# MasterBin-IIAU/UNINEXT

Measured on NVIDIA H100. Metric: msdeformattn_fwd_bwd_gsamples_per_s, higher is better.
Workload: dtype f32

## Files before the change

uninext_b200/csrc/msda_cabi.cu:

```cuda
#include <type_traits>

#include "../../include/msda_b200.h"
#include "msda_det.cuh"
#include "msda_generic.cuh"
#include "msda_host.cuh"
#include "msda_region.cuh"
#include "msda_slab.cuh"
#include "msda_tmem.cuh"
#include "msda_tiled.cuh"

std::atomic<uint64_t> msda_host::g_launches{0};

namespace {

using namespace msda_host;

struct Dims { int N, S, M, D, L, Lq, P; };

int check_dims(const Dims &d) {
    if (d.N <= 0 || d.S <= 0 || d.M <= 0 || d.D <= 0 || d.L <= 0 || d.Lq <= 0 || d.P <= 0) return MSDA_E_BADARG;
    if ((long long)d.S >= (1ll << 30)) return MSDA_E_TOOLARGE;
    if ((long long)d.N * d.Lq * d.M >= (1ll << 40)) return MSDA_E_TOOLARGE;
    return 0;
}

struct Knobs {
    std::atomic<int> v[MSDA_KNOB_COUNT];
    std::atomic<int> epoch{1};
    Knobs() {
        v[MSDA_KNOB_SLAB].store(env_int("MSDA_SLAB", -1));
        v[MSDA_KNOB_BWD_WIN_ROWS].store(env_int("MSDA_BWD_WIN_ROWS", -1));
        v[MSDA_KNOB_BWD_LIST_CAP].store(env_int("MSDA_BWD_LIST_CAP", 48));
        v[MSDA_KNOB_FWD_SLAB_CTAS].store(env_int("MSDA_FWD_SLAB_CTAS", 2));
        v[MSDA_KNOB_F32_VEC8_FWD].store(env_int("MSDA_F32_VEC8_FWD", 0));
        v[MSDA_KNOB_F32_VEC8_BWD].store(env_int("MSDA_F32_VEC8_BWD", 0));
        v[MSDA_KNOB_BF16_FINE_ROWS].store(env_int("MSDA_BF16_FINE_ROWS", 0));
        v[MSDA_KNOB_BF16_PACKED_FWD].store(env_int("MSDA_BF16_PACKED_FWD", 0));
        v[MSDA_KNOB_ZERO_FILL].store(env_int("MSDA_ZERO_FILL", 2));
        v[MSDA_KNOB_REGION_BWD].store(env_int("MSDA_REGION_BWD", -1));
    }
};
Knobs &knobs() { static Knobs k; return k; }
int knob(int i) { return knobs().v[i].load(std::memory_order_relaxed); }

cudaError_t zero_fill(void *p, size_t bytes, cudaStream_t st, bool *pdl = nullptr) {
    if (pdl) *pdl = false;
    const int mode = knob(MSDA_KNOB_ZERO_FILL);
    if (mode <= 0 || bytes < (1u << 16) || !aligned16(p) || (bytes & 15u)) return cudaMemsetAsync(p, 0, bytes, st);
    const unsigned long long n16 = bytes >> 4;
    msda::msda_zero_fill<<<capped_grid((long long)n16, 256, 8), 256, 0, st>>>(static_cast<uint4 *>(p), n16);
    const cudaError_t err = cudaGetLastError();
    if (pdl && mode >= 2 && err == cudaSuccess) {
        cudaStreamCaptureStatus cap = cudaStreamCaptureStatusNone;
        *pdl = cudaStreamIsCapturing(st, &cap) == cudaSuccess && cap == cudaStreamCaptureStatusNone;
    }
    return err;
}

bool fast_ok(int dtype_bytes, int D, int L, int P) {
    if (L > msda::kMaxLevels || L * P > 32) return false;
    if (dtype_bytes == 4) return D == 16 || D == 32 || D == 64;
    if (dtype_bytes == 2) return D == 32 || D == 64;
    return false;
}

bool use_fast(int dtype_bytes, const Dims &d) {
    return fast_ok(dtype_bytes, d.D, d.L, d.P) && (long long)d.N * d.Lq * d.M < (1ll << 31);
}

unsigned num_pairs(const Dims &d) { return (unsigned)((long long)d.N * d.Lq * d.M); }

template <typename T, class F>
cudaError_t route_tiled(const Dims &d, F f) {
    using L16 = std::integral_constant<int, 16>;
    using L32 = std::integral_constant<int, 32>;
    const bool lp16 = d.L * d.P <= 16;
    switch (d.D) {
        case 16:
            if constexpr (sizeof(T) == 4) return lp16 ? f(L16{}, L16{}) : f(L16{}, L32{});
            break;
        case 32: return lp16 ? f(L32{}, L16{}) : f(L32{}, L32{});
        case 64: return lp16 ? f(std::integral_constant<int, 64>{}, L16{}) : f(std::integral_constant<int, 64>{}, L32{});
    }
    return cudaErrorInvalidValue;
}

template <typename K>
int resident_ctas(K kernel) {
    int per_sm = 0;
    if (cudaOccupancyMaxActiveBlocksPerMultiprocessor(&per_sm, kernel, msda::kTiledThreads, 0) != cudaSuccess || per_sm < 1)
        per_sm = 1;
    return per_sm * num_sms();
}

int allow_patches() {
    static const int v = env_flag("MSDA_PATCHES") == 1;
    return v;
}

bool use_tma_staging(const Dims &d) {
    static const bool off = env_flag("MSDA_NO_TMA") == 1;
    return !off && !allow_patches() && ((d.L * d.P) % 4 == 0);
}

bool use_split(unsigned npairs) {
    static const int force = env_flag("MSDA_SPLIT");
    if (force >= 0) return force == 1;
    return npairs <= (unsigned)num_sms() * 56u;
}

constexpr int kFwdMinCtas = 4, kBwdMinCtas = 2;


template <typename T> struct FwdVec { static constexpr int v = 16 / sizeof(T); };
template <typename T> struct BwdVec { static constexpr int v = 4; };

template <typename K, typename... Args>
cudaError_t launch_after_fill(K kern, int grid, size_t smem, cudaStream_t st, bool pdl, Args... args) {
    if (pdl) {
        cudaLaunchConfig_t cfg = {};
        cfg.gridDim = dim3((unsigned)grid);
        cfg.blockDim = dim3(msda::kTiledThreads);
        cfg.dynamicSmemBytes = smem;
        cfg.stream = st;
        cudaLaunchAttribute attr[1];
        attr[0].id = cudaLaunchAttributeProgrammaticStreamSerialization;
        attr[0].val.programmaticStreamSerializationAllowed = 1;
        cfg.attrs = attr;
        cfg.numAttrs = 1;
        const cudaError_t e = cudaLaunchKernelEx(&cfg, kern, args...);
        return e != cudaSuccess ? e : cudaGetLastError();
    }
    kern<<<grid, msda::kTiledThreads, smem, st>>>(args...);
    return cudaGetLastError();
}

template <typename K, typename... Args>
cudaError_t launch_tiled(K kern, PerDevice<int> &slots, unsigned npairs, unsigned iter_pairs, bool pdl, cudaStream_t st,
                         Args... args) {
    const unsigned n = (unsigned)slots.get([&](int) { return resident_ctas(kern); });
    const unsigned tiles_ub = (npairs + iter_pairs - 1) / iter_pairs;
    g_launches.fetch_add(1, std::memory_order_relaxed);
    return launch_after_fill(kern, (int)(tiles_ub < n ? tiles_ub : n), 0, st, pdl, args...);
}

template <typename T, int D, int LP_MAX, int VEC = FwdVec<T>::v>
cudaError_t launch_fwd(const T *value, const int64_t *shapes, const int64_t *lsi, const float *loc, const float *attn,
                       const Dims &d, T *out, cudaStream_t st) {
    using Shape = msda::TiledShape<VEC, D, LP_MAX, false>;
    constexpr bool kCanStage = (LP_MAX <= 16);
    constexpr bool kCanSplit = Shape::kCanSplit;
    constexpr bool kCanPack = sizeof(T) == 2 && VEC == 8;
    const unsigned npairs = num_pairs(d);
    const bool split = kCanSplit && use_split(npairs);
    const bool tma = !split && kCanStage && use_tma_staging(d);
    const bool packed = kCanPack && !split && knob(MSDA_KNOB_BF16_PACKED_FWD) == 1;
    static decltype(&msda::msda_fwd_tiled<T, VEC, D, LP_MAX, kFwdMinCtas, false, false>) const kern[] = {
        msda::msda_fwd_tiled<T, VEC, D, LP_MAX, kFwdMinCtas, false, kCanSplit>,
        msda::msda_fwd_tiled<T, VEC, D, LP_MAX, kFwdMinCtas, kCanStage, false>,
        msda::msda_fwd_tiled<T, VEC, D, LP_MAX, kFwdMinCtas, false, false>,
        msda::msda_fwd_tiled<T, VEC, D, LP_MAX, kFwdMinCtas, kCanStage, false, kCanPack>,
        msda::msda_fwd_tiled<T, VEC, D, LP_MAX, kFwdMinCtas, false, false, kCanPack>};
    static PerDevice<int> slots[5];
    const int k = split ? 0 : (packed ? 3 : 1) + (tma ? 0 : 1);
    return launch_tiled(kern[k], slots[k], npairs, split ? msda::TiledShape<VEC, D, LP_MAX, kCanSplit>::kIterPairs
                                                         : Shape::kIterPairs,
                        false, st, value, shapes, lsi, loc, attn, d.N, d.S, d.M, d.L, d.Lq, d.P, npairs, allow_patches(), out);
}

template <typename T, int D, int LP_MAX, int VEC = BwdVec<T>::v, bool NORED = false>
cudaError_t launch_bwd(const T *grad_out, const T *value, const int64_t *shapes, const int64_t *lsi, const float *loc,
                       const float *attn, const Dims &d, float *gv, float *gl, float *ga, bool pdl, cudaStream_t st) {
    using Shape = msda::TiledShape<VEC, D, LP_MAX, false>;
    constexpr bool kCanStage = (LP_MAX <= 16);
    constexpr bool kCanSplit = Shape::kCanSplit;
    const unsigned npairs = num_pairs(d);
    const bool split = kCanSplit && use_split(npairs);
    const bool tma = !split && kCanStage && use_tma_staging(d);
    static decltype(&msda::msda_bwd_tiled<T, VEC, D, LP_MAX, kBwdMinCtas, false, false, false, NORED>) const kern[] = {
        msda::msda_bwd_tiled<T, VEC, D, LP_MAX, kBwdMinCtas, false, kCanSplit, false, NORED>,
        msda::msda_bwd_tiled<T, VEC, D, LP_MAX, kBwdMinCtas, kCanStage, false, false, NORED>,
        msda::msda_bwd_tiled<T, VEC, D, LP_MAX, kBwdMinCtas, false, false, false, NORED>};
    static PerDevice<int> slots[3];
    const int k = split ? 0 : tma ? 1 : 2;
    return launch_tiled(kern[k], slots[k], npairs, split ? msda::TiledShape<VEC, D, LP_MAX, kCanSplit>::kIterPairs
                                                         : Shape::kIterPairs,
                        pdl, st, grad_out, value, shapes, lsi, loc, attn, d.N, d.S, d.M, d.L, d.Lq, d.P, npairs,
                        allow_patches(), gv, gl, ga, (__nv_bfloat16 *)nullptr, 0);
}


bool use_slab(const Dims &d, const void *value, const void *out) {
    if (d.D != 32 || d.L * d.P > 16 || d.L > msda::kMaxLevels) return false;
    if ((reinterpret_cast<uintptr_t>(value) & 31u) || !aligned16(out)) return false;
    return knob(MSDA_KNOB_SLAB) == 1;
}

template <typename T>
cudaError_t launch_fwd_slab(const T *value, const int64_t *shapes, const int64_t *lsi, const float *loc, const float *attn,
                            const Dims &d, T *out, cudaStream_t st) {
    const int sms = num_sms();
    if (knob(MSDA_KNOB_FWD_SLAB_CTAS) == 1)
        return launch(msda::msda_fwd_slab<T, 16, 1>, sms, msda::kSlabThreads, 0, st, value, shapes, lsi, loc, attn, d.N,
                      d.S, d.M, d.L, d.Lq, d.P, sms, out);
    return launch(msda::msda_fwd_slab<T, 16, 2>, sms * 2, msda::kSlabThreads, 0, st, value, shapes, lsi, loc, attn, d.N,
                  d.S, d.M, d.L, d.Lq, d.P, sms, out);
}

struct Window { int rows, cap; };

template <auto Kernel, class Smem, class Fit>
cudaError_t bwd_window(int cap_max, Smem smem, Fit fit, Window &w) {
    static PerDevice<uint64_t> cache;
    const uint64_t epoch = (uint32_t)knobs().epoch.load(std::memory_order_acquire);
    cudaError_t e = cudaSuccess;
    const uint64_t v = cache.get([&](int dev) -> uint64_t {
        int cap = knob(MSDA_KNOB_BWD_LIST_CAP) & ~1;
        if (cap < 8) cap = 8;
        if (cap > cap_max) cap = cap_max;
        int max_optin = 0;
        cudaDeviceGetAttribute(&max_optin, cudaDevAttrMaxSharedMemoryPerBlockOptin, dev);
        cudaFuncAttributes fa{};
        cudaFuncGetAttributes(&fa, Kernel);
        const long long fixed = (long long)smem(0, cap) + (long long)fa.sharedSizeBytes + 64;
        int rows = fit((int)((max_optin - fixed) / 128));
        if (rows < 0) rows = 0;
        if ((e = opt_in_smem<Kernel>((int)smem(rows, cap))) != cudaSuccess) return 0;
        return epoch << 32 | (uint64_t)rows << 16 | (uint64_t)cap;
    }, [&](uint64_t c) { return c >> 32 == epoch; });
    w = Window{(int)(v >> 16 & 0xffff), (int)(v & 0xffff)};
    return e;
}

template <typename T>
cudaError_t launch_bwd_slab(const T *grad_out, const T *value, const int64_t *shapes, const int64_t *lsi, const float *loc,
                            const float *attn, const Dims &d, float *gv, float *gl, float *ga, cudaStream_t st) {
    constexpr auto kern = msda::msda_bwd_slab<T, 16>;
    const auto smem = [](int rows, int cap) { return msda::bwd_slab_smem_bytes(rows, cap); };
    Window w;
    const cudaError_t e = bwd_window<kern>(1 << 30, smem, [](int rows) {
        const int want = knob(MSDA_KNOB_BWD_WIN_ROWS);
        return want >= 0 && want < rows ? want : rows;
    }, w);
    if (e != cudaSuccess) return e;
    const int sms = num_sms();
    return launch(kern, sms, msda::kSlabThreads, smem(w.rows, w.cap), st, grad_out, value, shapes, lsi, loc, attn, d.N,
                  d.S, d.M, d.L, d.Lq, d.P, sms, w.rows, w.cap, gv, gl, ga);
}

cudaError_t launch_bwd_mixed(const __nv_bfloat16 *go, const __nv_bfloat16 *value, const int64_t *shapes, const int64_t *lsi,
                             const float *loc, const float *attn, const Dims &d, float *scratch, __nv_bfloat16 *gv16,
                             float *gl, float *ga, int fine_min_rows, cudaStream_t st) {
    using T = __nv_bfloat16;
    constexpr int VEC = 4, DD = 32, LP_MAX = 16;
    const unsigned npairs = num_pairs(d);
    static decltype(&msda::msda_bwd_tiled<T, VEC, DD, LP_MAX, kBwdMinCtas, false, false, true>) const kern[] = {
        msda::msda_bwd_tiled<T, VEC, DD, LP_MAX, kBwdMinCtas, true, false, true>,
        msda::msda_bwd_tiled<T, VEC, DD, LP_MAX, kBwdMinCtas, false, false, true>};
    static PerDevice<int> slots[2];
    const int k = use_tma_staging(d) ? 0 : 1;
    return launch_tiled(kern[k], slots[k], npairs, msda::TiledShape<VEC, DD, LP_MAX, false>::kIterPairs, false, st, go,
                        value, shapes, lsi, loc, attn, d.N, d.S, d.M, d.L, d.Lq, d.P, npairs, allow_patches(), scratch,
                        gl, ga, gv16, fine_min_rows);
}

template <typename T>
cudaError_t launch_bwd_tmem(const T *grad_out, const T *value, const int64_t *shapes, const int64_t *lsi, const float *loc,
                            const float *attn, const Dims &d, float *gv, float *gl, float *ga, cudaStream_t st) {
    constexpr auto kern = msda::msda_bwd_tmem<T, 16>;
    const auto smem = [](int rows, int cap) { return msda::bwd_tmem_smem_bytes(cap, rows); };
    Window w;
    const cudaError_t e = bwd_window<kern>(128, smem, [](int rows) { return rows & ~(msda::kTmCons - 1); }, w);
    if (e != cudaSuccess) return e;
    const int sms = num_sms();
    return launch(kern, sms, msda::kTmThreads, smem(w.rows, w.cap), st, grad_out, value, shapes, lsi, loc, attn, d.N, d.S,
                  d.M, d.L, d.Lq, d.P, sms, w.cap, w.rows, gv, gl, ga);
}

bool use_region(const Dims &d) {
    return knob(MSDA_KNOB_REGION_BWD) != 0 && d.D == 32 && d.L * d.P <= 16 && d.L <= msda::kMaxLevels && d.Lq == d.S &&
           !use_split(num_pairs(d));
}

cudaError_t launch_bwd_region(const float *go, const float *value, const int64_t *shapes, const int64_t *lsi,
                              const float *loc, const float *attn, const Dims &d, float *gv, float *gl, float *ga,
                              bool pdl, cudaStream_t st) {
    constexpr auto tap = msda::msda_bwd_region<msda::kRegionEdge, msda::kRegionHalo>;
    constexpr auto gvk = msda::msda_region_grad_value_pass<msda::kRegionEdge, msda::kRegionHalo>;
    constexpr size_t tap_smem = msda::region_tap_smem_bytes(), gv_smem = msda::region_gv_smem_bytes();
    if (const cudaError_t e = opt_in_smem<gvk>((int)gv_smem)) return e;
    const auto resident = [](auto kern, size_t smem) {
        int per_sm = 0;
        if (cudaOccupancyMaxActiveBlocksPerMultiprocessor(&per_sm, kern, msda::kTiledThreads, smem) != cudaSuccess || per_sm < 1)
            per_sm = 1;
        return per_sm * num_sms();
    };
    static PerDevice<int> tap_slots, gv_slots;
    const int tap_grid = tap_slots.get([&](int) { return resident(tap, tap_smem); });
    const int gv_grid = gv_slots.get([&](int) { return resident(gvk, gv_smem); });
    const unsigned npairs = num_pairs(d);
    const int tma = use_tma_staging(d) ? 1 : 0;
    g_launches.fetch_add(2, std::memory_order_relaxed);
    cudaError_t e = launch_after_fill(tap, tap_grid, tap_smem, st, pdl, go, value, shapes, lsi, loc, attn, d.N, d.S, d.M,
                                      d.L, d.Lq, d.P, npairs, tma, gl, ga);
    if (e != cudaSuccess) return e;
    cudaStreamCaptureStatus cap = cudaStreamCaptureStatusNone;
    const bool chain = cudaStreamIsCapturing(st, &cap) == cudaSuccess && cap == cudaStreamCaptureStatusNone;
    return launch_after_fill(gvk, gv_grid, gv_smem, st, chain, go, shapes, lsi, loc, attn, d.N, d.S, d.M, d.L, d.Lq, d.P,
                             npairs, gv);
}

template <typename T>
cudaError_t fwd_fast(const T *value, const int64_t *shapes, const int64_t *lsi, const float *loc, const float *attn,
                     const Dims &d, T *out, cudaStream_t st) {
    if (use_slab(d, value, out)) return launch_fwd_slab<T>(value, shapes, lsi, loc, attn, d, out, st);
    if constexpr (sizeof(T) == 4) {
        if (knob(MSDA_KNOB_F32_VEC8_FWD) == 1 && d.L * d.P <= 16 && (d.D == 32 || d.D == 64) &&
            !(reinterpret_cast<uintptr_t>(value) & 31u))
            return d.D == 32 ? launch_fwd<T, 32, 16, 8>(value, shapes, lsi, loc, attn, d, out, st)
                             : launch_fwd<T, 64, 16, 8>(value, shapes, lsi, loc, attn, d, out, st);
    }
    return route_tiled<T>(d, [&](auto D, auto LP) {
        return launch_fwd<T, decltype(D)::value, decltype(LP)::value>(value, shapes, lsi, loc, attn, d, out, st);
    });
}

template <typename T>
cudaError_t bwd_fast(const T *go, const T *value, const int64_t *shapes, const int64_t *lsi, const float *loc,
                     const float *attn, const Dims &d, float *gv, float *gl, float *ga, bool pdl, cudaStream_t st) {
    const int LP = d.L * d.P;
    if (knob(MSDA_KNOB_SLAB) == 2 && d.D == 32 && LP <= 16 && d.L <= msda::kMaxLevels)
        return launch_bwd_tmem<T>(go, value, shapes, lsi, loc, attn, d, gv, gl, ga, st);
    if (use_slab(d, value, gv)) return launch_bwd_slab<T>(go, value, shapes, lsi, loc, attn, d, gv, gl, ga, st);
    if constexpr (sizeof(T) == 4) {
        if (knob(MSDA_KNOB_F32_VEC8_BWD) == 1 && LP <= 16 && d.D == 32 &&
            !((reinterpret_cast<uintptr_t>(value) | reinterpret_cast<uintptr_t>(go)) & 31u))
            return launch_bwd<T, 32, 16, 8>(go, value, shapes, lsi, loc, attn, d, gv, gl, ga, pdl, st);
        if (use_region(d)) return launch_bwd_region(go, value, shapes, lsi, loc, attn, d, gv, gl, ga, pdl, st);
    }
    return route_tiled<T>(d, [&](auto D, auto LPM) {
        return launch_bwd<T, decltype(D)::value, decltype(LPM)::value>(go, value, shapes, lsi, loc, attn, d, gv, gl, ga,
                                                                       pdl, st);
    });
}

template <typename T, typename TL>
cudaError_t fwd_generic(const T *value, const int64_t *shapes, const int64_t *lsi, const TL *loc, const TL *attn,
                        const Dims &d, T *out, cudaStream_t st) {
    const long long total = (long long)d.N * d.Lq * d.M * d.D;
    return launch(msda::msda_fwd_generic<T, TL>, capped_grid(total, 256, 32), 256, 0, st, value, shapes, lsi, loc, attn,
                  d.S, d.M, d.D, d.L, d.Lq, d.P, total, out);
}

template <typename T, typename TL, typename GA, bool NORED = false>
cudaError_t bwd_generic(const T *go, const T *value, const int64_t *shapes, const int64_t *lsi, const TL *loc,
                        const TL *attn, const Dims &d, GA *gv, TL *gl, TL *ga, cudaStream_t st) {
    const long long npairs = (long long)d.N * d.Lq * d.M;
    int threads = ((d.D + 31) / 32) * 32;
    if (threads > 256) threads = 256;
    return launch(msda::msda_bwd_generic<T, TL, GA, NORED>, capped_grid(npairs, 1, 64), threads, 0, st, go, value, shapes,
                  lsi, loc, attn, d.S, d.M, d.D, d.L, d.Lq, d.P, npairs, gv, gl, ga);
}

cudaError_t round_to_bf16(const float *gv32, uint16_t *gv, size_t nval, cudaStream_t st) {
    return launch(msda::msda_f32_to_bf16, capped_grid((long long)nval, 256, 16), 256, 0, st, gv32,
                  reinterpret_cast<__nv_bfloat16 *>(gv), (long long)nval);
}

template <class A> struct Elem { using type = A; };
template <> struct Elem<uint16_t> { using type = __nv_bfloat16; };

#define MSDA_CHECK_PTRS(ALIGNED, ...)                                    \
    bool ALIGNED = true;                                                 \
    do {                                                                 \
        const void *ptrs_[] = {__VA_ARGS__};                             \
        for (const void *p_ : ptrs_) {                                   \
            if (p_ == nullptr) return MSDA_E_BADARG;                     \
            ALIGNED = ALIGNED && aligned16(p_);                          \
        }                                                                \
    } while (0)

template <class A, class TL>
int forward(const A *value, const int64_t *shapes, const int64_t *lsi, const TL *loc, const TL *attn, const Dims &d, A *out,
            void *stream) {
    using T = typename Elem<A>::type;
    if (int e = check_dims(d)) return e;
    MSDA_CHECK_PTRS(al, value, loc, attn, out);
    if (!shapes || !lsi) return MSDA_E_BADARG;
    cudaStream_t st = static_cast<cudaStream_t>(stream);
    const T *v = reinterpret_cast<const T *>(value);
    T *o = reinterpret_cast<T *>(out);
    if constexpr (sizeof(T) != 8)
        if (al && use_fast(sizeof(T), d)) return (int)fwd_fast<T>(v, shapes, lsi, loc, attn, d, o, st);
    return (int)fwd_generic<T, TL>(v, shapes, lsi, loc, attn, d, o, st);
}

int backward_mixed(const __nv_bfloat16 *go, const __nv_bfloat16 *v, const int64_t *shapes, const int64_t *lsi,
                   const float *loc, const float *attn, const Dims &d, float *gv32, uint16_t *gv, float *gl, float *ga,
                   int fine_rows, cudaStream_t st) {
    __nv_bfloat16 *gv16 = reinterpret_cast<__nv_bfloat16 *>(gv);
    cudaError_t e = zero_fill(gv, sizeof(uint16_t) * (size_t)d.N * d.S * d.M * d.D, st);
    if (e != cudaSuccess) return (int)e;
    const dim3 hgrid((unsigned)(num_sms() * 2 / d.N + 1), (unsigned)d.N);
    if ((e = launch(msda::msda_coarse_rows<false>, hgrid, 256, 0, st, gv32, gv16, shapes, lsi, d.L, d.S, d.M * d.D,
                    fine_rows)) != cudaSuccess)
        return (int)e;
    e = launch_bwd_mixed(go, v, shapes, lsi, loc, attn, d, gv32, gv16, gl, ga, fine_rows, st);
    if (e != cudaSuccess) return (int)e;
    return (int)launch(msda::msda_coarse_rows<true>, hgrid, 256, 0, st, gv32, gv16, shapes, lsi, d.L, d.S, d.M * d.D,
                       fine_rows);
}

template <class A, class TL, class C>
int backward(const A *grad_out, const A *value, const int64_t *shapes, const int64_t *lsi, const TL *loc, const TL *attn,
             const Dims &d, C *gv, uint16_t *gv16, TL *gl, TL *ga, void *stream) {
    using T = typename Elem<A>::type;
    if (int e = check_dims(d)) return e;
    MSDA_CHECK_PTRS(al, grad_out, value, loc, attn, gv, gl, ga);
    if (!shapes || !lsi) return MSDA_E_BADARG;
    cudaStream_t st = static_cast<cudaStream_t>(stream);
    const size_t nval = (size_t)d.N * d.S * d.M * d.D;
    const T *go = reinterpret_cast<const T *>(grad_out), *v = reinterpret_cast<const T *>(value);
    const bool fast = al && use_fast(sizeof(T), d);
    if constexpr (sizeof(T) == 2) {
        const int fine_rows = knob(MSDA_KNOB_BF16_FINE_ROWS);
        if (fine_rows > 0 && gv16 != nullptr && fast && d.D == 32 && d.L * d.P <= 16 && !use_split(num_pairs(d)) &&
            aligned16(gv16))
            return backward_mixed(go, v, shapes, lsi, loc, attn, d, gv, gv16, gl, ga, fine_rows, st);
    }
    bool pdl = false;
    cudaError_t err = zero_fill(gv, sizeof(C) * nval, st, sizeof(T) != 8 ? &pdl : nullptr);
    if (err != cudaSuccess) return (int)err;
    if constexpr (sizeof(T) != 8) {
        if (fast) err = bwd_fast<T>(go, v, shapes, lsi, loc, attn, d, gv, gl, ga, pdl, st);
    }
    if (!fast) err = bwd_generic<T, TL, C>(go, v, shapes, lsi, loc, attn, d, gv, gl, ga, st);
    if constexpr (sizeof(T) == 2) {
        if (err == cudaSuccess && gv16 != nullptr) err = round_to_bf16(gv, gv16, nval, st);
    }
    return (int)err;
}


struct DetLayout { size_t keys_in, keys_out, vals_in, vals_out, start, counter, temp, temp_bytes, total; unsigned n; };

int det_end_bit(const Dims &d) {
    const unsigned long long top = (unsigned long long)d.M * d.S;
    int bits = 0;
    while (bits < 32 && (top >> bits) != 0) ++bits;
    return bits;
}

int det_layout(const Dims &d, long long nq, DetLayout &lay) {
    const unsigned long long n = (unsigned long long)nq * d.M * d.L * d.P * 4;
    if (n > 0xffffffffull) return MSDA_E_TOOLARGE;
    lay.n = (unsigned)n;
    size_t off = 0;
    auto take = [&](size_t bytes) { const size_t at = off; off += align256(bytes); return at; };
    lay.keys_in = take(4 * n);
    lay.keys_out = take(4 * n);
    lay.vals_in = take(4 * n);
    lay.vals_out = take(4 * n);
    lay.start = take(4 * ((size_t)d.M * d.S + 1));
    lay.counter = take(4);
    lay.temp_bytes = 0;
    const cudaError_t e = msda::det_sort(nullptr, lay.temp_bytes, nullptr, nullptr, nullptr, nullptr, lay.n, det_end_bit(d), 0);
    if (e != cudaSuccess) return (int)e;
    lay.temp = take(lay.temp_bytes);
    lay.total = off;
    return 0;
}

int det_check(const Dims &d) {
    if (int e = check_dims(d)) return e;
    if ((unsigned long long)d.M * d.S + 1 > (1ull << 32)) return MSDA_E_TOOLARGE;
    return 0;
}

template <typename T, typename TL, typename GA>
cudaError_t det_loc_attn(const T *go, const T *value, const int64_t *shapes, const int64_t *lsi, const TL *loc,
                         const TL *attn, const Dims &d, bool fast, GA *gv, TL *gl, TL *ga, cudaStream_t st) {
    if constexpr (sizeof(T) != 8) {
        if (fast)
            return route_tiled<T>(d, [&](auto D, auto LP) {
                return launch_bwd<T, decltype(D)::value, decltype(LP)::value, 4, true>(go, value, shapes, lsi, loc, attn, d,
                                                                                       gv, gl, ga, false, st);
            });
    }
    return bwd_generic<T, TL, GA, true>(go, value, shapes, lsi, loc, attn, d, gv, gl, ga, st);
}

template <typename T, typename TL>
int det_backward(const T *go, const T *value, const int64_t *shapes, const int64_t *lsi, const TL *loc, const TL *attn,
                 const Dims &d, bool fast, typename msda::Num<T>::C *gv, TL *gl, TL *ga, void *ws, int64_t ws_bytes,
                 cudaStream_t st) {
    using C = typename msda::Num<T>::C;
    if (ws == nullptr || ws_bytes <= 0) return MSDA_E_BADARG;
    DetLayout lay{};
    if (int e = det_layout(d, 1, lay)) return e;
    if ((long long)lay.total > ws_bytes) return MSDA_E_BADARG;
    long long lo = 1, hi = d.Lq;
    while (lo < hi) {
        const long long mid = hi - (hi - lo) / 2;
        DetLayout t{};
        const int e = det_layout(d, mid, t);
        if (e == 0 && (long long)t.total <= ws_bytes) lo = mid; else if (e != 0 && e != MSDA_E_TOOLARGE) return e; else hi = mid - 1;
    }
    const long long chunk = lo;
    cudaError_t err = cudaMemsetAsync(gv, 0, sizeof(C) * (size_t)d.N * d.S * d.M * d.D, st);
    if (err != cudaSuccess) return (int)err;
    err = det_loc_attn<T, TL, C>(go, value, shapes, lsi, loc, attn, d, fast, gv, gl, ga, st);
    if (err != cudaSuccess) return (int)err;

    unsigned char *w = static_cast<unsigned char *>(ws);
    const int end_bit = det_end_bit(d);
    const unsigned nkeys = (unsigned)d.M * (unsigned)d.S;
    const bool v4 = sizeof(T) != 8 && d.D == 32 && fast;
    const int sms = num_sms();
    const int LP = d.L * d.P;
    for (int b = 0; b < d.N; ++b) {
        for (long long q0 = 0; q0 < d.Lq; q0 += chunk) {
            const long long nq = q0 + chunk <= d.Lq ? chunk : d.Lq - q0;
            if (int e = det_layout(d, nq, lay)) return e;
            unsigned *keys_in = reinterpret_cast<unsigned *>(w + lay.keys_in), *keys_out = reinterpret_cast<unsigned *>(w + lay.keys_out);
            unsigned *vals_in = reinterpret_cast<unsigned *>(w + lay.vals_in), *vals_out = reinterpret_cast<unsigned *>(w + lay.vals_out);
            unsigned *start = reinterpret_cast<unsigned *>(w + lay.start), *counter = reinterpret_cast<unsigned *>(w + lay.counter);
            const long long tap0 = ((long long)b * d.Lq + q0) * d.M * LP;
            const T *go_chunk = go + ((size_t)b * d.Lq + q0) * d.M * d.D;
            msda::msda_det_keys<TL><<<capped_grid(lay.n, msda::kDetThreads, 16), msda::kDetThreads, 0, st>>>(
                loc, shapes, lsi, d.S, d.M, d.L, d.P, tap0, lay.n, keys_in, vals_in);
            if ((err = cudaGetLastError()) != cudaSuccess) return (int)err;
            size_t temp_bytes = lay.temp_bytes;
            err = msda::det_sort(w + lay.temp, temp_bytes, keys_in, keys_out, vals_in, vals_out, lay.n, end_bit, st);
            if (err != cudaSuccess) return (int)err;
            msda::msda_det_bounds<<<capped_grid((long long)nkeys + 1, msda::kDetThreads, 16), msda::kDetThreads, 0, st>>>(
                keys_out, lay.n, nkeys, start);
            if ((err = cudaGetLastError()) != cudaSuccess) return (int)err;
            if ((err = cudaMemsetAsync(counter, 0, 4, st)) != cudaSuccess) return (int)err;
            if constexpr (sizeof(T) != 8) {
                if (v4) {
                    msda::msda_det_accumulate_v4<T><<<sms * 8, msda::kDetThreads, 0, st>>>(
                        go_chunk, loc, attn, shapes, d.S, d.M, d.L, d.P, tap0, b, start, vals_out, counter, gv);
                }
            }
            if (!v4)
                msda::msda_det_accumulate<T, TL><<<sms * 8, msda::kDetThreads, 0, st>>>(
                    go_chunk, loc, attn, shapes, d.S, d.M, d.D, d.L, d.P, tap0, b, start, vals_out, counter, gv);
            if ((err = cudaGetLastError()) != cudaSuccess) return (int)err;
            g_launches.fetch_add(4, std::memory_order_relaxed);
        }
    }
    return 0;
}

template <class A, class TL, class C>
int det_entry(const A *grad_out, const A *value, const int64_t *shapes, const int64_t *lsi, const TL *loc, const TL *attn,
              const Dims &d, C *gv, uint16_t *gv16, TL *gl, TL *ga, void *ws, int64_t ws_bytes, void *stream) {
    using T = typename Elem<A>::type;
    if (int e = det_check(d)) return e;
    MSDA_CHECK_PTRS(al, grad_out, value, loc, attn, gv, gl, ga);
    if (!shapes || !lsi) return MSDA_E_BADARG;
    cudaStream_t st = static_cast<cudaStream_t>(stream);
    const int e = det_backward<T, TL>(reinterpret_cast<const T *>(grad_out), reinterpret_cast<const T *>(value), shapes,
                                      lsi, loc, attn, d, al && use_fast(sizeof(T), d), gv, gl, ga, ws, ws_bytes, st);
    if constexpr (sizeof(T) == 2) {
        if (e == 0 && gv16 != nullptr) return (int)round_to_bf16(gv, gv16, (size_t)d.N * d.S * d.M * d.D, st);
    }
    return e;
}

}

extern "C" {

int msda_abi_version(void) { return MSDA_ABI_VERSION; }

const char *msda_strerror(int code) {
    if (code == 0) return "success";
    if (code == MSDA_E_BADARG) return "msda: bad argument (null pointer, non-positive dimension or unknown knob)";
    if (code == MSDA_E_TOOLARGE) return "msda: problem too large for the kernel index types";
    if (code == MSDA_E_NODEVICE) return "msda: no CUDA device";
    if (code > 0) return cudaGetErrorString(static_cast<cudaError_t>(code));
    return "msda: unknown error";
}

int msda_uses_fast_path(int dtype_bytes, int D, int L, int P) { return fast_ok(dtype_bytes, D, L, P) ? 1 : 0; }

uint64_t msda_launch_count(void) { return g_launches.load(std::memory_order_relaxed); }

int msda_set_knob(int k, int value) {
    if (k < 0 || k >= MSDA_KNOB_COUNT) return MSDA_E_BADARG;
    Knobs &kn = knobs();
    if (value == MSDA_KNOB_QUERY) return kn.v[k].load(std::memory_order_relaxed);
    const int old = kn.v[k].exchange(value, std::memory_order_relaxed);
    kn.epoch.fetch_add(1, std::memory_order_release);
    return old;
}

int msda_forward_f32(const float *value, const int64_t *spatial_shapes, const int64_t *level_start_index,
                     const float *sampling_loc, const float *attn_weight, int N, int S, int M, int D, int L, int Lq,
                     int P, float *out, void *stream) {
    return forward(value, spatial_shapes, level_start_index, sampling_loc, attn_weight, {N, S, M, D, L, Lq, P}, out, stream);
}

int msda_forward_f64(const double *value, const int64_t *spatial_shapes, const int64_t *level_start_index,
                     const double *sampling_loc, const double *attn_weight, int N, int S, int M, int D, int L, int Lq,
                     int P, double *out, void *stream) {
    return forward(value, spatial_shapes, level_start_index, sampling_loc, attn_weight, {N, S, M, D, L, Lq, P}, out, stream);
}

int msda_forward_bf16(const uint16_t *value, const int64_t *spatial_shapes, const int64_t *level_start_index,
                      const float *sampling_loc, const float *attn_weight, int N, int S, int M, int D, int L, int Lq,
                      int P, uint16_t *out, void *stream) {
    return forward(value, spatial_shapes, level_start_index, sampling_loc, attn_weight, {N, S, M, D, L, Lq, P}, out, stream);
}

int msda_backward_f32(const float *grad_out, const float *value, const int64_t *spatial_shapes,
                      const int64_t *level_start_index, const float *sampling_loc, const float *attn_weight, int N,
                      int S, int M, int D, int L, int Lq, int P, float *grad_value, float *grad_sampling_loc,
                      float *grad_attn_weight, void *stream) {
    return backward(grad_out, value, spatial_shapes, level_start_index, sampling_loc, attn_weight, {N, S, M, D, L, Lq, P},
                    grad_value, nullptr, grad_sampling_loc, grad_attn_weight, stream);
}

int msda_backward_f64(const double *grad_out, const double *value, const int64_t *spatial_shapes,
                      const int64_t *level_start_index, const double *sampling_loc, const double *attn_weight, int N,
                      int S, int M, int D, int L, int Lq, int P, double *grad_value, double *grad_sampling_loc,
                      double *grad_attn_weight, void *stream) {
    return backward(grad_out, value, spatial_shapes, level_start_index, sampling_loc, attn_weight, {N, S, M, D, L, Lq, P},
                    grad_value, nullptr, grad_sampling_loc, grad_attn_weight, stream);
}

int msda_backward_bf16(const uint16_t *grad_out, const uint16_t *value, const int64_t *spatial_shapes,
                       const int64_t *level_start_index, const float *sampling_loc, const float *attn_weight, int N,
                       int S, int M, int D, int L, int Lq, int P, float *grad_value_f32, uint16_t *grad_value,
                       float *grad_sampling_loc, float *grad_attn_weight, void *stream) {
    return backward(grad_out, value, spatial_shapes, level_start_index, sampling_loc, attn_weight, {N, S, M, D, L, Lq, P},
                    grad_value_f32, grad_value, grad_sampling_loc, grad_attn_weight, stream);
}

int msda_backward_det_workspace(int dtype_bytes, int N, int S, int M, int D, int L, int Lq, int P, int chunk_queries,
                                int64_t *bytes) {
    const Dims d{N, S, M, D, L, Lq, P};
    if (dtype_bytes != 2 && dtype_bytes != 4 && dtype_bytes != 8) return MSDA_E_BADARG;
    if (!bytes || chunk_queries <= 0) return MSDA_E_BADARG;
    if (int e = det_check(d)) return e;
    DetLayout lay{};
    if (int e = det_layout(d, chunk_queries < Lq ? chunk_queries : Lq, lay)) return e;
    *bytes = (int64_t)lay.total;
    return 0;
}

int msda_backward_det_f32(const float *grad_out, const float *value, const int64_t *spatial_shapes,
                          const int64_t *level_start_index, const float *sampling_loc, const float *attn_weight, int N,
                          int S, int M, int D, int L, int Lq, int P, float *grad_value, float *grad_sampling_loc,
                          float *grad_attn_weight, void *workspace, int64_t workspace_bytes, void *stream) {
    return det_entry(grad_out, value, spatial_shapes, level_start_index, sampling_loc, attn_weight, {N, S, M, D, L, Lq, P},
                     grad_value, nullptr, grad_sampling_loc, grad_attn_weight, workspace, workspace_bytes, stream);
}

int msda_backward_det_f64(const double *grad_out, const double *value, const int64_t *spatial_shapes,
                          const int64_t *level_start_index, const double *sampling_loc, const double *attn_weight, int N,
                          int S, int M, int D, int L, int Lq, int P, double *grad_value, double *grad_sampling_loc,
                          double *grad_attn_weight, void *workspace, int64_t workspace_bytes, void *stream) {
    return det_entry(grad_out, value, spatial_shapes, level_start_index, sampling_loc, attn_weight, {N, S, M, D, L, Lq, P},
                     grad_value, nullptr, grad_sampling_loc, grad_attn_weight, workspace, workspace_bytes, stream);
}

int msda_backward_det_bf16(const uint16_t *grad_out, const uint16_t *value, const int64_t *spatial_shapes,
                           const int64_t *level_start_index, const float *sampling_loc, const float *attn_weight, int N,
                           int S, int M, int D, int L, int Lq, int P, float *grad_value_f32, uint16_t *grad_value,
                           float *grad_sampling_loc, float *grad_attn_weight, void *workspace, int64_t workspace_bytes,
                           void *stream) {
    return det_entry(grad_out, value, spatial_shapes, level_start_index, sampling_loc, attn_weight, {N, S, M, D, L, Lq, P},
                     grad_value_f32, grad_value, grad_sampling_loc, grad_attn_weight, workspace, workspace_bytes, stream);
}

}
```

uninext_b200/csrc/msda_region.cuh:

```cuda
#pragma once

#include "msda_tiled.cuh"

namespace msda {

constexpr int kRegionEdge = 8;
constexpr int kRegionHalo = 2;
constexpr int kRegionSlots = 96;
constexpr int kRegionWinRows = 1024;
constexpr int kRegionStageRows = 384;
constexpr int kRegionEntries = kRegionSlots * 16 * 4;
constexpr int kRegionTapCtas = 2;
constexpr int kRegionGvCtas = 3;
constexpr int kRegionIterSlots = kTiledWarps * 4;

using RegionTapStage = TapStage<4, 16, true>;

constexpr size_t region_tap_smem_bytes() { return (size_t)kTiledWarps * RegionTapStage::kBytes; }

constexpr size_t region_gv_smem_bytes() {
    static_assert(kRegionEntries <= 0x10000, "entry indices are u16");
    return (size_t)kRegionEntries * (4 + 2 + 2) + (size_t)kRegionSlots * 128 + (size_t)kRegionWinRows * 4;
}

#ifdef MSDA_REGION_PHASE_CLOCKS
constexpr int kRegionSpans = 4;
__device__ unsigned long long *g_region_clocks;
__device__ int g_region_knockout;
#define MSDA_REGION_CLOCK_INIT long long region_clk = clock64()
#define MSDA_REGION_CLOCK(span)                                                                  \
    if (threadIdx.x == 0) {                                                                      \
        const long long now = clock64();                                                         \
        g_region_clocks[blockIdx.x * kRegionSpans + (span)] += (unsigned long long)(now - region_clk); \
        region_clk = now;                                                                        \
    }
#define MSDA_REGION_KEEP_RED(bit) (!(g_region_knockout & (bit)))
#else
#define MSDA_REGION_CLOCK_INIT
#define MSDA_REGION_CLOCK(span)
#define MSDA_REGION_KEEP_RED(bit) true
#endif

struct RegionMap {
    int H[kMaxLevels], W[kMaxLevels], start[kMaxLevels];
    int Href, Wref, nry, nrx;
    int region;
    unsigned ntiles;
};

struct RegionTile {
    int b, m, nq, nwin;
    unsigned base_pair;
    int qy0[kMaxLevels], qx0[kMaxLevels], qny[kMaxLevels], qnx[kMaxLevels], qpre[kMaxLevels + 1];
    int wy0[kMaxLevels], wx0[kMaxLevels], wh[kMaxLevels], ww[kMaxLevels], wbase[kMaxLevels + 1];
};

__device__ __forceinline__ int region_first(int r, int n, int ref, int R) {
    const long long num = 2ll * r * n * R - ref;
    return num <= 0 ? 0 : (int)min((long long)n, (num + 2ll * ref - 1) / (2ll * ref));
}

template <int R, int HALO>
__global__ void __launch_bounds__(kTiledThreads, kRegionGvCtas)
msda_region_grad_value_pass(const float *__restrict__ grad_out, const int64_t *__restrict__ shapes,
                            const int64_t *__restrict__ lsi, const float *__restrict__ loc,
                            const float *__restrict__ attn, int N, int S, int M, int L, int Lq, int P, unsigned npairs,
                            float *__restrict__ grad_value)
{
    constexpr int D = 32, VEC = 4, LPR = D / VEC, GPW = 32 / LPR, LP_MAX = 16, NSL = LP_MAX / LPR;
    static_assert(GPW * kTiledWarps == kRegionIterSlots && kRegionSlots <= 256 && kRegionWinRows < 0xffff &&
                  kRegionSlots % kRegionIterSlots == 0, "entry layout");
    constexpr unsigned short kNoRow = 0xffff;

    __shared__ RegionMap rm;
    __shared__ RegionTile tl;
    __shared__ int wsum[kTiledWarps];
    __shared__ __align__(16) unsigned char slab_mem[kTiledWarps * TapSlab<LPR>::kBytes];
    extern __shared__ __align__(128) unsigned char region_dyn[];
    float *e_coef = reinterpret_cast<float *>(region_dyn);
    float4 *gstash = reinterpret_cast<float4 *>(e_coef + kRegionEntries);
    int *cnt = reinterpret_cast<int *>(gstash + kRegionSlots * LPR);
    unsigned short *e_row = reinterpret_cast<unsigned short *>(cnt + kRegionWinRows);
    unsigned short *s_idx = e_row + kRegionEntries;

    MSDA_REGION_CLOCK_INIT;
    if (threadIdx.x == 0) {
        int run = 0, href = 0, wref = 0;
        bool tiled = (Lq == S);
        for (int l = 0; l < L; ++l) {
            const int h = (int)shapes[2 * l], w = (int)shapes[2 * l + 1], st = (int)lsi[l];
            rm.H[l] = h; rm.W[l] = w; rm.start[l] = st;
            tiled = tiled && (st == run) && h > 0 && w > 0;
            run += h * w;
            href = max(href, h); wref = max(wref, w);
        }
        tiled = tiled && (run == S);
        rm.region = tiled ? 1 : 0;
        rm.Href = href; rm.Wref = wref;
        rm.nry = (href + R - 1) / R; rm.nrx = (wref + R - 1) / R;
        rm.ntiles = tiled ? (unsigned)N * (unsigned)M * (unsigned)(rm.nry * rm.nrx)
                          : (npairs + kRegionIterSlots - 1) / kRegionIterSlots;
    }
    __syncthreads();

    const int lane = threadIdx.x & 31, warp = threadIdx.x >> 5;
    const int sub = lane % LPR, grp = lane / LPR;
    const int LP = L * P;
    const unsigned row_elems = (unsigned)(M * D);
    TapSlab<LPR> slab(slab_mem + warp * TapSlab<LPR>::kBytes, grp);
    bool primary_done = false;
    for (unsigned tile = blockIdx.x; tile < rm.ntiles; tile += gridDim.x) {
        if (rm.region) {
            const int m = (int)(tile % (unsigned)M);
            const unsigned r = tile / (unsigned)M, per_b = (unsigned)(rm.nry * rm.nrx);
            const int reg = (int)(r % per_b), ry = reg / rm.nrx, rx = reg % rm.nrx;
            const int l = threadIdx.x;
            if (l < L) {
                const int H = rm.H[l], W = rm.W[l];
                const int y0 = region_first(ry, H, rm.Href, R), y1 = region_first(ry + 1, H, rm.Href, R);
                const int x0 = region_first(rx, W, rm.Wref, R), x1 = region_first(rx + 1, W, rm.Wref, R);
                tl.qy0[l] = y0; tl.qny[l] = y1 - y0; tl.qx0[l] = x0; tl.qnx[l] = x1 - x0;
                const int wy0 = max(0, (int)((long long)ry * R * H / rm.Href) - HALO);
                const int wy1 = min(H, (int)(((long long)(ry + 1) * R * H + rm.Href - 1) / rm.Href) + HALO);
                const int wx0 = max(0, (int)((long long)rx * R * W / rm.Wref) - HALO);
                const int wx1 = min(W, (int)(((long long)(rx + 1) * R * W + rm.Wref - 1) / rm.Wref) + HALO);
                tl.wy0[l] = wy0; tl.wh[l] = wy1 - wy0; tl.wx0[l] = wx0; tl.ww[l] = wx1 - wx0;
            }
            if (threadIdx.x == 0) { tl.m = m; tl.b = (int)(r / per_b); }
            __syncthreads();
            if (threadIdx.x == 0) {
                int nq = 0, nw = 0;
                for (int k = 0; k < L; ++k) {
                    tl.qpre[k] = nq; nq += tl.qny[k] * tl.qnx[k];
                    const int rows = tl.wh[k] * tl.ww[k];
                    if (nw + rows > kRegionWinRows) { tl.wh[k] = tl.ww[k] = 0; }
                    tl.wbase[k] = nw; nw += tl.wh[k] * tl.ww[k];
                }
                tl.qpre[L] = nq; tl.wbase[L] = nw;
                tl.nq = nq; tl.nwin = nw;
            }
        } else if (threadIdx.x == 0) {
            tl.base_pair = tile * kRegionIterSlots;
            tl.nq = (int)min((unsigned)kRegionIterSlots, npairs - tl.base_pair);
            tl.nwin = 0;
        }
        __syncthreads();
        for (int i = threadIdx.x; i < tl.nwin; i += kTiledThreads) cnt[i] = 0;
        __syncthreads();
        MSDA_REGION_CLOCK(0);

#pragma unroll 1
        for (int it = 0; it * kRegionIterSlots < tl.nq; ++it) {
            const int slot = it * kRegionIterSlots + warp * GPW + grp;
            const bool active = slot < tl.nq;
            unsigned pair = 0; int b = 0, m = 0;
            if (active) {
                if (rm.region) {
                    int l = 0;
                    while (l + 1 < L && slot >= tl.qpre[l + 1]) ++l;
                    const int k = slot - tl.qpre[l], y = tl.qy0[l] + k / tl.qnx[l], x = tl.qx0[l] + k % tl.qnx[l];
                    b = tl.b; m = tl.m;
                    pair = ((unsigned)b * (unsigned)Lq + (unsigned)(rm.start[l] + y * rm.W[l] + x)) * (unsigned)M + (unsigned)m;
                } else {
                    pair = tl.base_pair + (unsigned)slot;
                    m = (int)(pair % (unsigned)M);
                    b = (int)((pair / (unsigned)M) / (unsigned)Lq);
                }
            }
            const bool stash = rm.region && active && slot < kRegionSlots;

            float g[VEC] = {0.f, 0.f, 0.f, 0.f};
            if (active) RowVec<float, VEC>::load(grad_out + (size_t)pair * D + (size_t)sub * VEC, g);
            if (stash) gstash[slot * LPR + sub] = make_float4(g[0], g[1], g[2], g[3]);

            float4 tw[NSL];
            int2 tr[NSL];
#pragma unroll
            for (int k = 0; k < NSL; ++k) {
                const int s = sub + k * LPR;
                tw[k] = make_float4(0.f, 0.f, 0.f, 0.f);
                tr[k] = make_int2(0, 0);
                unsigned filed = 0;
                ushort4 rows4 = make_ushort4(kNoRow, kNoRow, kNoRow, kNoRow);
                float4 w4 = make_float4(0.f, 0.f, 0.f, 0.f);
                if (s < LP && active) {
                    const size_t t = (size_t)pair * LP + s;
                    const float2 xy = __ldg(reinterpret_cast<const float2 *>(loc) + t);
                    const float a = __ldg(attn + t);
                    const int l = s / P;
                    const TapGeom gm = tap_geometry(xy.x, xy.y, rm.H[l], rm.W[l], rm.start[l]);
                    w4 = masked_weights(gm, a);
                    tr[k] = make_int2(gm.r0, gm.r1 | (gm.dw << 31));
                    const unsigned nz = (unsigned)(w4.x != 0.f) | ((unsigned)(w4.y != 0.f) << 1) |
                                        ((unsigned)(w4.z != 0.f) << 2) | ((unsigned)(w4.w != 0.f) << 3);
                    if (stash) {
                        const int W = rm.W[l], o0 = gm.r0 - rm.start[l], o1 = gm.r1 - rm.start[l];
                        const int y0 = o0 / W, x0 = o0 - y0 * W, y1 = o1 / W;
                        const int wwl = tl.ww[l], whl = tl.wh[l];
                        const int ry0 = y0 - tl.wy0[l], ry1 = y1 - tl.wy0[l], rx0 = x0 - tl.wx0[l], rx1 = rx0 + gm.dw;
                        const unsigned iy0 = (unsigned)ry0 < (unsigned)whl, iy1 = (unsigned)ry1 < (unsigned)whl;
                        const unsigned ix0 = (unsigned)rx0 < (unsigned)wwl, ix1 = (unsigned)rx1 < (unsigned)wwl;
                        const unsigned inwin = (iy0 & ix0) | ((iy0 & ix1) << 1) | ((iy1 & ix0) << 2) | ((iy1 & ix1) << 3);
                        filed = inwin & nz;
                        const int w00 = tl.wbase[l] + ry0 * wwl + rx0, dhw = (y1 - y0) * wwl;
                        const int wr[4] = {w00, w00 + gm.dw, w00 + dhw, w00 + dhw + gm.dw};
#pragma unroll
                        for (int c = 0; c < 4; ++c)
                            if ((filed >> c) & 1u) atomicAdd(&cnt[wr[c]], 1);
                        rows4 = make_ushort4((filed & 1u) ? (unsigned short)wr[0] : kNoRow,
                                             (filed & 2u) ? (unsigned short)wr[1] : kNoRow,
                                             (filed & 4u) ? (unsigned short)wr[2] : kNoRow,
                                             (filed & 8u) ? (unsigned short)wr[3] : kNoRow);
                    }
                    tw[k] = make_float4((filed & 1u) ? 0.f : w4.x, (filed & 2u) ? 0.f : w4.y,
                                        (filed & 4u) ? 0.f : w4.z, (filed & 8u) ? 0.f : w4.w);
                }
                if (stash) {
                    const int e = (slot * LP_MAX + s) << 2;
                    *reinterpret_cast<ushort4 *>(e_row + e) = rows4;
                    *reinterpret_cast<float4 *>(e_coef + e) = w4;
                }
            }

            if (!primary_done) {
                pdl_wait_primary();
                primary_done = true;
            }
            const size_t slab_off = ((size_t)b * S * M + m) * D + (size_t)sub * VEC;
            float *gbase = grad_value + slab_off;
#pragma unroll
            for (int k = 0; k < NSL; ++k) {
                __syncwarp();
                slab.put(sub, tw[k], tr[k]);
                __syncwarp();
                const bool any = tw[k].x != 0.f || tw[k].y != 0.f || tw[k].z != 0.f || tw[k].w != 0.f;
                unsigned todo = (__ballot_sync(kFullMask, any) >> (grp * LPR)) & ((1u << LPR) - 1u);
                while (todo) {
                    const int j = __ffs(todo) - 1;
                    todo &= todo - 1u;
                    const float4 w4 = slab.weights(j);
                    const int2 rr = slab.rows(j);
                    const float w[4] = {w4.x, w4.y, w4.z, w4.w};
                    const unsigned dwo = (rr.y < 0) ? row_elems : 0u;
                    unsigned long long off[4];
                    off[0] = (unsigned long long)(unsigned)rr.x * row_elems;
                    off[1] = off[0] + dwo;
                    off[2] = (unsigned long long)(unsigned)(rr.y & 0x7fffffff) * row_elems;
                    off[3] = off[2] + dwo;
#pragma unroll
                    for (int c = 0; c < 4; ++c)
                        if (w[c] != 0.f && MSDA_REGION_KEEP_RED(1))
                            red_add_v4(gbase + off[c], w[c] * g[0], w[c] * g[1], w[c] * g[2], w[c] * g[3]);
                }
            }
        }

        const int nwin = tl.nwin;
        if (nwin > 0) {
            __syncthreads();
            MSDA_REGION_CLOCK(1);
            const int n = min(tl.nq, kRegionSlots) * LP_MAX * 4;
            {
                const int i0 = threadIdx.x * 4;
                int c[4], sum = 0;
#pragma unroll
                for (int q = 0; q < 4; ++q) { c[q] = (i0 + q < nwin) ? cnt[i0 + q] : 0; sum += c[q]; }
                int incl = sum;
#pragma unroll
                for (int d = 1; d < 32; d <<= 1) {
                    const int t = __shfl_up_sync(kFullMask, incl, d);
                    if (lane >= d) incl += t;
                }
                if (lane == 31) wsum[warp] = incl;
                __syncthreads();
                int run = incl - sum;
                for (int w = 0; w < warp; ++w) run += wsum[w];
#pragma unroll
                for (int q = 0; q < 4; ++q)
                    if (i0 + q < nwin) { cnt[i0 + q] = run; run += c[q]; }
            }
            static_assert(kRegionWinRows <= 4 * kTiledThreads, "scan covers 4 rows per thread");
            __syncthreads();
            for (int e = threadIdx.x; e < n; e += kTiledThreads) {
                const unsigned short r = e_row[e];
                if (r != kNoRow) s_idx[atomicAdd(&cnt[r], 1)] = (unsigned short)e;
            }
            __syncthreads();
            MSDA_REGION_CLOCK(2);

            const int b = tl.b, m = tl.m;
            for (int r = warp * GPW + grp; r < nwin; r += kRegionIterSlots) {
                const int beg = r ? cnt[r - 1] : 0, end = cnt[r];
                if (beg == end) continue;
                float4 acc = make_float4(0.f, 0.f, 0.f, 0.f);
#pragma unroll 4
                for (int i = beg; i < end; ++i) {
                    const int e = s_idx[i];
                    const float cf = e_coef[e];
                    const float4 gs = gstash[(e / (LP_MAX * 4)) * LPR + sub];
                    acc.x = fmaf(cf, gs.x, acc.x); acc.y = fmaf(cf, gs.y, acc.y);
                    acc.z = fmaf(cf, gs.z, acc.z); acc.w = fmaf(cf, gs.w, acc.w);
                }
                int l = 0;
                while (l + 1 < L && r >= tl.wbase[l + 1]) ++l;
                const int k = r - tl.wbase[l], y = tl.wy0[l] + k / tl.ww[l], x = tl.wx0[l] + k % tl.ww[l];
                const int row = rm.start[l] + y * rm.W[l] + x;
                if (MSDA_REGION_KEEP_RED(2))
                    red_add_v4(grad_value + (((size_t)b * S + row) * M + m) * D + (size_t)sub * VEC, acc.x, acc.y, acc.z, acc.w);
            }
        }
        __syncthreads();
        MSDA_REGION_CLOCK(nwin > 0 ? 3 : 1);
    }
}

template <int R, int HALO>
__global__ void __launch_bounds__(kTiledThreads, kRegionTapCtas)
msda_bwd_region(const float *__restrict__ grad_out, const float *__restrict__ value,
                const int64_t *__restrict__ shapes, const int64_t *__restrict__ lsi,
                const float *__restrict__ loc, const float *__restrict__ attn,
                int N, int S, int M, int L, int Lq, int P, unsigned npairs, int tma,
                float *__restrict__ grad_loc, float *__restrict__ grad_attn)
{
    __shared__ WorkMap wm;
    __shared__ __align__(16) unsigned char slab_mem[kTiledWarps * TapSlab<8>::kBytes];
    __shared__ __align__(8) unsigned long long stage_bar[kTiledWarps * 2];
    extern __shared__ __align__(128) unsigned char stage_mem[];

    pdl_launch_dependents();
    if (tma)
        bwd_tiled_body<float, 4, 32, 16, true, false, false, true, false>(
            wm, slab_mem, stage_mem, stage_bar, grad_out, value, shapes, lsi, loc, attn, N, S, M, L, Lq, P, npairs, 0,
            nullptr, grad_loc, grad_attn, nullptr, 0);
    else
        bwd_tiled_body<float, 4, 32, 16, false, false, false, true, false>(
            wm, slab_mem, stage_mem, stage_bar, grad_out, value, shapes, lsi, loc, attn, N, S, M, L, Lq, P, npairs, 0,
            nullptr, grad_loc, grad_attn, nullptr, 0);
    pdl_wait_primary();
}

}
```

Baseline: 5.494.

## Co-schedule region grad-value and tap kernels via PDL with occupancy-sized grids

Swaps the launch order of the two region backward kernels so the grad-value pass runs first and triggers PDL early. The tap kernel then launches as a dependent and can run alongside it on the same SMs. A helper picks a grad-value grid size and padded dynamic shared memory so that one tap CTA per SM fits next to the grad-value CTAs. The goal is to overlap the two kernels instead of running them back to back, at the cost of possibly lower grad-value occupancy. It also adds optional co-scheduling timing instrumentation.

```diff
diff --git a/uninext_b200/csrc/msda_cabi.cu b/uninext_b200/csrc/msda_cabi.cu
--- a/uninext_b200/csrc/msda_cabi.cu
+++ b/uninext_b200/csrc/msda_cabi.cu
@@ -288,26 +288,28 @@
     constexpr auto tap = msda::msda_bwd_region<msda::kRegionEdge, msda::kRegionHalo>;
     constexpr auto gvk = msda::msda_region_grad_value_pass<msda::kRegionEdge, msda::kRegionHalo>;
     constexpr size_t tap_smem = msda::region_tap_smem_bytes(), gv_smem = msda::region_gv_smem_bytes();
-    if (const cudaError_t e = opt_in_smem<gvk>((int)gv_smem)) return e;
-    const auto resident = [](auto kern, size_t smem) {
-        int per_sm = 0;
-        if (cudaOccupancyMaxActiveBlocksPerMultiprocessor(&per_sm, kern, msda::kTiledThreads, smem) != cudaSuccess || per_sm < 1)
-            per_sm = 1;
-        return per_sm * num_sms();
-    };
-    static PerDevice<int> tap_slots, gv_slots;
-    const int tap_grid = tap_slots.get([&](int) { return resident(tap, tap_smem); });
-    const int gv_grid = gv_slots.get([&](int) { return resident(gvk, gv_smem); });
+    static PerDevice<int> ready;
+    static msda::RegionGrids grids[kMaxDevices];
+    cudaError_t e = cudaSuccess;
+    const int dev = current_device();
+    ready.get([&](int dv) {
+        if ((e = cudaFuncSetAttribute(gvk, cudaFuncAttributeMaxDynamicSharedMemorySize, (int)gv_smem)) != cudaSuccess)
+            return 0;
+        grids[dv] = msda::region_grids(gvk, gv_smem, tap, tap_smem, num_sms());
+        return 1;
+    });
+    if (e != cudaSuccess) return e;
+    const msda::RegionGrids &rg = grids[dev];
+    cudaStreamCaptureStatus cap = cudaStreamCaptureStatusNone;
+    const bool chain = cudaStreamIsCapturing(st, &cap) == cudaSuccess && cap == cudaStreamCaptureStatusNone;
     const unsigned npairs = num_pairs(d);
     const int tma = use_tma_staging(d) ? 1 : 0;
     g_launches.fetch_add(2, std::memory_order_relaxed);
-    cudaError_t e = launch_after_fill(tap, tap_grid, tap_smem, st, pdl, go, value, shapes, lsi, loc, attn, d.N, d.S, d.M,
-                                      d.L, d.Lq, d.P, npairs, tma, gl, ga);
+    e = launch_after_fill(gvk, chain ? rg.gv : rg.gv_solo, chain ? rg.gv_smem : gv_smem, st, pdl, go, shapes, lsi, loc,
+                          attn, d.N, d.S, d.M, d.L, d.Lq, d.P, npairs, gv);
     if (e != cudaSuccess) return e;
-    cudaStreamCaptureStatus cap = cudaStreamCaptureStatusNone;
-    const bool chain = cudaStreamIsCapturing(st, &cap) == cudaSuccess && cap == cudaStreamCaptureStatusNone;
-    return launch_after_fill(gvk, gv_grid, gv_smem, st, chain, go, shapes, lsi, loc, attn, d.N, d.S, d.M, d.L, d.Lq, d.P,
-                             npairs, gv);
+    return launch_after_fill(tap, chain ? rg.tap : rg.tap_solo, tap_smem, st, chain, go, value, shapes, lsi, loc, attn, d.N,
+                             d.S, d.M, d.L, d.Lq, d.P, npairs, tma, gl, ga);
 }
 
 template <typename T>
diff --git a/uninext_b200/csrc/msda_region.cuh b/uninext_b200/csrc/msda_region.cuh
--- a/uninext_b200/csrc/msda_region.cuh
+++ b/uninext_b200/csrc/msda_region.cuh
@@ -41,6 +41,28 @@
 #define MSDA_REGION_KEEP_RED(bit) true
 #endif
 
+#ifdef MSDA_REGION_COSCHED
+__device__ unsigned long long *g_region_cosched[2];
+__device__ __forceinline__ unsigned long long region_globaltimer() {
+    unsigned long long t;
+    asm volatile("mov.u64 %0, %%globaltimer;" : "=l"(t));
+    return t;
+}
+#define MSDA_REGION_COSCHED_START(k)                                                               \
+    if (threadIdx.x == 0) {                                                                        \
+        unsigned smid;                                                                             \
+        asm volatile("mov.u32 %0, %%smid;" : "=r"(smid));                                         \
+        g_region_cosched[k][3 * blockIdx.x] = smid;                                                \
+        g_region_cosched[k][3 * blockIdx.x + 1] = region_globaltimer();                            \
+    }
+#define MSDA_REGION_COSCHED_END(k)                                                                 \
+    __syncthreads();                                                                               \
+    if (threadIdx.x == 0) g_region_cosched[k][3 * blockIdx.x + 2] = region_globaltimer();
+#else
+#define MSDA_REGION_COSCHED_START(k)
+#define MSDA_REGION_COSCHED_END(k)
+#endif
+
 struct RegionMap {
     int H[kMaxLevels], W[kMaxLevels], start[kMaxLevels];
     int Href, Wref, nry, nrx;
@@ -83,6 +105,8 @@
     unsigned short *e_row = reinterpret_cast<unsigned short *>(cnt + kRegionWinRows);
     unsigned short *s_idx = e_row + kRegionEntries;
 
+    pdl_launch_dependents();
+    MSDA_REGION_COSCHED_START(0);
     MSDA_REGION_CLOCK_INIT;
     if (threadIdx.x == 0) {
         int run = 0, href = 0, wref = 0;
@@ -312,6 +336,8 @@
         __syncthreads();
         MSDA_REGION_CLOCK(nwin > 0 ? 3 : 1);
     }
+    if (!primary_done) pdl_wait_primary();
+    MSDA_REGION_COSCHED_END(0);
 }
 
 template <int R, int HALO>
@@ -327,7 +353,7 @@
     __shared__ __align__(8) unsigned long long stage_bar[kTiledWarps * 2];
     extern __shared__ __align__(128) unsigned char stage_mem[];
 
-    pdl_launch_dependents();
+    MSDA_REGION_COSCHED_START(1);
     if (tma)
         bwd_tiled_body<float, 4, 32, 16, true, false, false, true, false>(
             wm, slab_mem, stage_mem, stage_bar, grad_out, value, shapes, lsi, loc, attn, N, S, M, L, Lq, P, npairs, 0,
@@ -336,7 +362,57 @@
         bwd_tiled_body<float, 4, 32, 16, false, false, false, true, false>(
             wm, slab_mem, stage_mem, stage_bar, grad_out, value, shapes, lsi, loc, attn, N, S, M, L, Lq, P, npairs, 0,
             nullptr, grad_loc, grad_attn, nullptr, 0);
+    MSDA_REGION_COSCHED_END(1);
     pdl_wait_primary();
 }
 
-}
+struct RegionGrids {
+    int gv, tap;
+    size_t gv_smem;
+    int gv_solo, tap_solo;
+};
+
+template <class GV, class TAP>
+RegionGrids region_grids(GV gvk, size_t gv_smem, TAP tap, size_t tap_smem, int sms) {
+    const auto occupancy = [](auto kern, size_t smem) {
+        int per_sm = 0;
+        if (cudaOccupancyMaxActiveBlocksPerMultiprocessor(&per_sm, kern, kTiledThreads, smem) != cudaSuccess || per_sm < 1)
+            per_sm = 1;
+        return per_sm;
+    };
+    const int gv_occ = occupancy(gvk, gv_smem), tap_occ = occupancy(tap, tap_smem);
+    const RegionGrids solo = {gv_occ * sms, tap_occ * sms, gv_smem, gv_occ * sms, tap_occ * sms};
+    int dev = 0, regs_sm = 0, smem_sm = 0, smem_optin = 0, reserved = 0, threads_sm = 0;
+    cudaFuncAttributes ga{}, ta{};
+    if (cudaGetDevice(&dev) != cudaSuccess ||
+        cudaDeviceGetAttribute(&regs_sm, cudaDevAttrMaxRegistersPerMultiprocessor, dev) != cudaSuccess ||
+        cudaDeviceGetAttribute(&smem_sm, cudaDevAttrMaxSharedMemoryPerMultiprocessor, dev) != cudaSuccess ||
+        cudaDeviceGetAttribute(&smem_optin, cudaDevAttrMaxSharedMemoryPerBlockOptin, dev) != cudaSuccess ||
+        cudaDeviceGetAttribute(&reserved, cudaDevAttrReservedSharedMemoryPerBlock, dev) != cudaSuccess ||
+        cudaDeviceGetAttribute(&threads_sm, cudaDevAttrMaxThreadsPerMultiProcessor, dev) != cudaSuccess ||
+        cudaFuncGetAttributes(&ga, gvk) != cudaSuccess || cudaFuncGetAttributes(&ta, tap) != cudaSuccess)
+        return solo;
+    constexpr int warps = kTiledThreads / 32;
+    const auto regs = [](int per_thread) { return warps * ((per_thread * 32 + 255) / 256 * 256); };
+    const auto smem = [&](const cudaFuncAttributes &a, size_t dyn) { return (long long)a.sharedSizeBytes + (long long)dyn + reserved; };
+    for (int g = gv_occ; g >= 1; --g) {
+        size_t dyn = gv_smem;
+        if (g < gv_occ) {
+            const long long over = (long long)smem_sm / (g + 1) + 1 - smem(ga, 0);
+            dyn = (size_t)((over + 1023) / 1024 * 1024);
+        }
+        if ((long long)g * regs(ga.numRegs) + regs(ta.numRegs) <= regs_sm && (long long)dyn <= smem_optin &&
+            g * smem(ga, dyn) + smem(ta, tap_smem) <= smem_sm && (g + 1) * kTiledThreads <= threads_sm) {
+            if (dyn != gv_smem &&
+                (cudaFuncSetAttribute(gvk, cudaFuncAttributeMaxDynamicSharedMemorySize, (int)dyn) != cudaSuccess ||
+                 cudaFuncSetAttribute(gvk, cudaFuncAttributePreferredSharedMemoryCarveout,
+                                      (int)cudaSharedmemCarveoutMaxShared) != cudaSuccess ||
+                 occupancy(gvk, dyn) != g))
+                return solo;
+            return {g * sms, sms, dyn, solo.gv_solo, solo.tap_solo};
+        }
+    }
+    return solo;
+}
+
+}
```

Result: faster. 5.986 (median of 6 runs) (+8.9%).
